# haoheliu/AudioLDM2

Hardware: AMD Instinct MI355X
Metric: audio_seconds_per_second (higher is better)
Workload: dtype f32 storage/accumulate; each product = 6 bf16 MFMA partial products of exact 3-part operand splits (fp32-grade); 1 GPU; audioldm2-full: batch 8 prompts/GPU x 1 GPU, 10.24 s @16 kHz, 200 DDIM steps, CFG 3.5, eta 1.0, n_candidates 1; one step = sample_log + VAE decode + HiFi-GAN + D2H of the waveform; synthetic conditioning, random-init weights, host-CPU RNG noise; global_batch=8, parallelism=prompt-sharded replicas x1, weight_broadcast_bytes=0

## Files before the change

### audioldm2_amd/csrc/api.hip

```cpp
#include "common.h"
#include <string.h>

namespace aldm {
static thread_local char g_err[512] = "";
void set_error(const char* fmt, ...) {
    va_list ap;
    va_start(ap, fmt);
    vsnprintf(g_err, sizeof(g_err), fmt, ap);
    va_end(ap);
}
}

extern "C" int aldm_version(void) { return 27; }
extern "C" const char* aldm_last_error(void) { return aldm::g_err; }
```

### audioldm2_amd/csrc/norm.hip

```cpp
#include <stdlib.h>
#include "igemm_epilogue.h"

namespace aldm {

constexpr int GN_ITERS = 16;
constexpr int GN_UNROLL = 8;

struct GnPart {
    float n, mean, m2;
};

__device__ __forceinline__ void gn_merge(double& n, double& mean, double& m2, double nb, double mb, double m2b) {
    if (nb <= 0.0) return;
    const double nt = n + nb;
    const double dlt = mb - mean;
    mean += dlt * (nb / nt);
    m2 += m2b + dlt * dlt * (n * nb / nt);
    n = nt;
}

template <bool FUSED>
__global__ __launch_bounds__(256) void gn_partial_kernel(const float* __restrict__ x1,
                                                         const float* __restrict__ x2, int P,
                                                         int C1, int C2, int G, int cols, int rows,
                                                         int chunk_px, float* __restrict__ ws, float eps,
                                                         const float* __restrict__ gamma,
                                                         const float* __restrict__ beta,
                                                         float* __restrict__ scale, float* __restrict__ shift, int gpb,
                                                         char* __restrict__ dst = nullptr, char* __restrict__ dst_raw = nullptr,
                                                         int parts = 3, int act = ALDM_ACT_NONE, int raw_parts = 3,
                                                         float f16_scale = 0.f) {
    const int C = C1 + C2;
    const int Cg4 = (C / G) >> 2;
    const int b = blockIdx.y;
    const int chunk = FUSED ? 0 : blockIdx.x;
    const int g_lo = FUSED ? blockIdx.x * gpb : 0;
    const int c4_lo = g_lo * Cg4, C4 = c4_lo + gpb * Cg4;
    const int p0 = chunk * chunk_px;
    const int p1 = min(P, p0 + chunk_px);
    const int tid = threadIdx.x;
    const int tx = tid % cols, ty = tid / cols;
    __shared__ GnPart ps[256];
    const int npass = (C4 - c4_lo + cols - 1) / cols;
    __shared__ double gacc[64][3];
    if (tid < 64) gacc[tid][0] = gacc[tid][1] = gacc[tid][2] = 0.0;
    __syncthreads();
    for (int cp = 0; cp < npass; ++cp) {
        const int c4 = c4_lo + cp * cols + tx;
        GnPart part = {0.f, 0.f, 0.f};
        if (ty < rows && c4 < C4 && p0 + ty < p1) {
            const int c = c4 << 2;
            const bool first = c < C1;
            const float* src = first ? x1 + (int64_t)b * P * C1 + c : x2 + (int64_t)b * P * C2 + (c - C1);
            const int pitch = first ? C1 : C2;
            float sa[GN_UNROLL], sq[GN_UNROLL];
#pragma unroll
            for (int u = 0; u < GN_UNROLL; ++u) sa[u] = sq[u] = 0.f;
            int p = p0 + ty;
            const f32x4 pv = *reinterpret_cast<const f32x4*>(src + (int64_t)p * pitch);
            const float pivot = fmaxf(fminf(pv[0], pv[1]), fminf(fmaxf(pv[0], pv[1]), pv[2]));
            int cnt = 0;
            for (; p + (GN_UNROLL - 1) * rows < p1; p += GN_UNROLL * rows) {
                f32x4 v[GN_UNROLL];
#pragma unroll
                for (int u = 0; u < GN_UNROLL; ++u)
                    v[u] = *reinterpret_cast<const f32x4*>(src + (int64_t)(p + u * rows) * pitch) - pivot;
#pragma unroll
                for (int u = 0; u < GN_UNROLL; ++u) {
                    sa[u] += (v[u][0] + v[u][1]) + (v[u][2] + v[u][3]);
                    sq[u] += (v[u][0] * v[u][0] + v[u][1] * v[u][1]) + (v[u][2] * v[u][2] + v[u][3] * v[u][3]);
                }
                cnt += GN_UNROLL;
            }
            for (; p < p1; p += rows) {
                const f32x4 v = *reinterpret_cast<const f32x4*>(src + (int64_t)p * pitch) - pivot;
                sa[0] += (v[0] + v[1]) + (v[2] + v[3]);
                sq[0] += (v[0] * v[0] + v[1] * v[1]) + (v[2] * v[2] + v[3] * v[3]);
                ++cnt;
            }
            float s = 0.f, ss = 0.f;
#pragma unroll
            for (int u = 0; u < GN_UNROLL; u += 2) {
                s += sa[u] + sa[u + 1];
                ss += sq[u] + sq[u + 1];
            }
            const float n = 4.0f * (float)cnt;
            const float md = s / n;
            part.n = n;
            part.mean = pivot + md;
            part.m2 = fmaxf(ss - s * md, 0.f);
        }
        if constexpr (FUSED) {
            __shared__ double wred[4][3];
            const int mygl = (c4 - c4_lo) / Cg4;
            for (int gl = 0; gl < gpb; ++gl) {
                const bool mine = part.n > 0.f && mygl == gl;
                double n = mine ? (double)part.n : 0.0, mean = mine ? (double)part.mean : 0.0, m2 = mine ? (double)part.m2 : 0.0;
#pragma unroll
                for (int o = 32; o > 0; o >>= 1) {
                    const double nb = __shfl_xor(n, o), mb = __shfl_xor(mean, o), m2b = __shfl_xor(m2, o);
                    gn_merge(n, mean, m2, nb, mb, m2b);
                }
                if ((tid & 63) == 0) {
                    wred[tid >> 6][0] = n;
                    wred[tid >> 6][1] = mean;
                    wred[tid >> 6][2] = m2;
                }
                __syncthreads();
                if (tid == 0) {
                    double an = gacc[gl][0], am = gacc[gl][1], a2 = gacc[gl][2];
                    for (int w = 0; w < 4; ++w) gn_merge(an, am, a2, wred[w][0], wred[w][1], wred[w][2]);
                    gacc[gl][0] = an;
                    gacc[gl][1] = am;
                    gacc[gl][2] = a2;
                }
                __syncthreads();
            }
            continue;
        }
        ps[tid] = part;
        __syncthreads();
        if (tid < gpb) {
            const int g = g_lo + tid;
            const int base = c4_lo + cp * cols;
            const int lo = max(g * Cg4, base), hi = min((g + 1) * Cg4, min(C4, base + cols));
            if (lo < hi) {
                double n = gacc[tid][0], mean = gacc[tid][1], m2 = gacc[tid][2];
                for (int yy = 0; yy < rows; ++yy)
                    for (int cc = lo; cc < hi; ++cc) {
                        const GnPart& t = ps[yy * cols + (cc - base)];
                        gn_merge(n, mean, m2, (double)t.n, (double)t.mean, (double)t.m2);
                    }
                gacc[tid][0] = n;
                gacc[tid][1] = mean;
                gacc[tid][2] = m2;
            }
        }
        __syncthreads();
    }
    if (FUSED) {
        const int Cg = C / G;
        __shared__ float fin[64][2];
        if (tid < gpb) {
            const double n = gacc[tid][0];
            double var = n > 0.0 ? gacc[tid][2] / n : 0.0;
            if (var < 0.0) var = 0.0;
            fin[tid][0] = (float)gacc[tid][1];
            fin[tid][1] = (float)(1.0 / sqrt(var + (double)eps));
        }
        __syncthreads();
        __shared__ float lsc[256], lsh[256];
        for (int c = g_lo * Cg + tid; c < (g_lo + gpb) * Cg; c += 256) {
            const int g = c / Cg - g_lo;
            const float sc = fin[g][1] * (gamma ? gamma[c] : 1.f);
            const float sh = (beta ? beta[c] : 0.f) - fin[g][0] * sc;
            scale[(int64_t)b * C + c] = sc;
            shift[(int64_t)b * C + c] = sh;
            if (dst) {
                lsc[c - g_lo * Cg] = sc;
                lsh[c - g_lo * Cg] = sh;
            }
        }
        if (dst) {
            __syncthreads();
            const int c_lo = g_lo * Cg, sw = (gpb * Cg) >> 3;
            for (int i = tid; i < P * sw; i += 256) {
                const int p = i / sw;
                const int cl = (i - p * sw) << 3;
                const int c = c_lo + cl;
                const int64_t row = (int64_t)b * P + p;
                const float* src = c < C1 ? x1 + row * C1 + c : x2 + row * C2 + (c - C1);
                f32x4 v0 = *reinterpret_cast<const f32x4*>(src);
                f32x4 v1 = *reinterpret_cast<const f32x4*>(src + 4);
                const int64_t off = (row * (C >> 5) + (c >> 5)) * (64 * parts) + (c & 31) * 2;
                u32x2 p0[3], p1[3];
                if (dst_raw) {
                    const int64_t roff = (row * (C >> 5) + (c >> 5)) * (64 * raw_parts) + (c & 31) * 2;
                    split4_parts(v0, p0, raw_parts);
                    split4_parts(v1, p1, raw_parts);
#pragma unroll
                    for (int q = 0; q < 3; ++q)
                        if (q < raw_parts)
                            *reinterpret_cast<u32x4*>(dst_raw + roff + q * 64) = u32x4{p0[q][0], p0[q][1], p1[q][0], p1[q][1]};
                }
#pragma unroll
                for (int e = 0; e < 4; ++e) {
                    v0[e] = __builtin_fmaf(v0[e], lsc[cl + e], lsh[cl + e]);
                    v1[e] = __builtin_fmaf(v1[e], lsc[cl + 4 + e], lsh[cl + 4 + e]);
                }
                if (act == ALDM_ACT_SILU) {
#pragma unroll
                    for (int e = 0; e < 4; ++e) {
                        v0[e] = silu_fast(v0[e]);
                        v1[e] = silu_fast(v1[e]);
                    }
                }
                split4_fmt(v0, p0, parts, f16_scale);
                split4_fmt(v1, p1, parts, f16_scale);
#pragma unroll
                for (int q = 0; q < 3; ++q)
                    if (q < parts) *reinterpret_cast<u32x4*>(dst + off + q * 64) = u32x4{p0[q][0], p0[q][1], p1[q][0], p1[q][1]};
            }
        }
    } else if (tid < G) {
// ... 217 lines not shown
        pl.cols = c4b < 256 ? c4b : 256;
        pl.rows = 256 / pl.cols;
        pl.chunk_px = P;
        pl.chunks = 1;
        pl.passes = (c4b + pl.cols - 1) / pl.cols;
    } else {
        pl.form = ALDM_GN_CHUNKED;
        gn_geometry(P, C, &pl.cols, &pl.rows, &pl.chunk_px, &pl.chunks);
        pl.passes = (C / 4 + pl.cols - 1) / pl.cols;
    }
    const int px = P < pl.chunk_px ? P : pl.chunk_px;
    pl.active = pl.cols * (pl.rows < px ? pl.rows : px);
    return pl;
}

}

using namespace aldm;

extern "C" int64_t aldm_gn_ws_floats(int B, int P, int C, int G) {
    int cols, rows, chunk_px, chunks;
    gn_geometry(P, C, &cols, &rows, &chunk_px, &chunks);
    return (int64_t)B * chunks * G * 6 + 2;
}

extern "C" int aldm_split_rows(const float* x1, const float* x2, int C1, int C2, int64_t rows, int P, const float* scale,
                               const float* shift, int act, void* dst, void* dst_raw, int parts, void* stream);
extern "C" int aldm_split_rows_f16(const float* x1, const float* x2, int C1, int C2, int64_t rows, int P, const float* scale,
                                   const float* shift, int act, float slope, void* dst, void* dst_raw, int raw_parts, float f16_scale,
                                   void* stream);

extern "C" int aldm_groupnorm_plan(int B, int P, int C1, int C2, int G, int want_split, int* form, int* group_slices,
                                   int* groups_per_block, int* chunks, int* chunk_px, int* cols, int* rows, int* passes,
                                   int* active_threads) {
    const int C = C1 + C2;
    ALDM_CHECK(B > 0 && P > 0 && C1 > 0 && C2 >= 0, "aldm_groupnorm_plan: bad shape (B=%d P=%d C1=%d C2=%d)", B, P, C1, C2);
    ALDM_CHECK(G > 0 && G <= 64 && C % G == 0 && (C / G) % 4 == 0 && C1 % 4 == 0,
               "aldm_groupnorm_plan: need C%%G==0, (C/G)%%4==0, C1%%4==0 (C1=%d C2=%d G=%d)", C1, C2, G);
    ALDM_CHECK(!want_split || (C % 32 == 0 && C1 % 8 == 0 && C2 % 8 == 0),
               "aldm_groupnorm_plan: a split image needs (C1+C2) %% 32 == 0, C1 %% 8 == 0 (C1=%d C2=%d)", C1, C2);
    const GnPlan pl = groupnorm_plan(B, P, C, C1, G, want_split != 0);
    if (form) *form = pl.form;
    if (group_slices) *group_slices = pl.gs;
    if (groups_per_block) *groups_per_block = pl.gpb;
    if (chunks) *chunks = pl.chunks;
    if (chunk_px) *chunk_px = pl.chunk_px;
    if (cols) *cols = pl.cols;
    if (rows) *rows = pl.rows;
    if (passes) *passes = pl.passes;
    if (active_threads) *active_threads = pl.active;
    return 0;
}

static int groupnorm_launch(const float* x1, const float* x2, int B, int P, int C1, int C2, int G, float eps,
                            const float* gamma, const float* beta, float* scale, float* shift, float* ws, void* dst,
                            void* dst_raw, int parts, int act, void* stream, int raw_parts = 0, float f16_scale = 0.f) {
    if (raw_parts == 0) raw_parts = parts;
    if (!x2) C2 = 0;
    const int C = C1 + C2;
    ALDM_CHECK(x1 && scale && shift && ws, "aldm_groupnorm_stats: null pointer");
    ws = reinterpret_cast<float*>((reinterpret_cast<uintptr_t>(ws) + 7) & ~uintptr_t(7));
    ALDM_CHECK(G > 0 && G <= 64 && C % G == 0 && (C / G) % 4 == 0 && C1 % 4 == 0,
               "aldm_groupnorm_stats: need C%%G==0, (C/G)%%4==0, C1%%4==0 (C1=%d C2=%d G=%d)", C1, C2, G);
    const GnPlan pl = groupnorm_plan(B, P, C, C1, G, dst != nullptr);
    hipStream_t st = (hipStream_t)stream;
    if (pl.form == ALDM_GN_FUSED_SPLIT) {
        hipLaunchKernelGGL(gn_partial_kernel<true>, dim3(pl.gs, B), dim3(256), 0, st, x1, x2, P, C1, C2, G, pl.cols, pl.rows, P, ws,
                           eps, gamma, beta, scale, shift, pl.gpb, reinterpret_cast<char*>(dst),
                           reinterpret_cast<char*>(dst_raw), parts, act, raw_parts, f16_scale);
        ALDM_LAUNCH_CHECK("aldm_groupnorm_split");
        return 0;
    }
    if (pl.form == ALDM_GN_FUSED) {
        hipLaunchKernelGGL(gn_partial_kernel<true>, dim3(pl.gs, B), dim3(256), 0, st, x1, x2, P, C1, C2, G, pl.cols,
                           pl.rows, P, ws, eps, gamma, beta, scale, shift, pl.gpb, nullptr, nullptr, 3, ALDM_ACT_NONE);
    } else {
        hipLaunchKernelGGL(gn_partial_kernel<false>, dim3(pl.chunks, B), dim3(256), 0, st, x1, x2, P, C1, C2, G,
                           pl.cols, pl.rows, pl.chunk_px, ws, eps, gamma, beta, scale, shift, G);
        hipLaunchKernelGGL(gn_finalize_kernel, dim3(B), dim3(256), 0, st, ws, pl.chunks, P, C, G, eps, gamma,
                           beta, scale, shift);
    }
    ALDM_LAUNCH_CHECK("aldm_groupnorm_stats");
    if (dst) {
        if (f16_scale != 0.f)
            return aldm_split_rows_f16(x1, x2, C1, C2, (int64_t)B * P, P, scale, shift, act, 0.f, dst, dst_raw, raw_parts, f16_scale, stream);
        return aldm_split_rows(x1, x2, C1, C2, (int64_t)B * P, P, scale, shift, act, dst, dst_raw, parts, stream);
    }
    return 0;
}

extern "C" int aldm_groupnorm_stats(const float* x1, const float* x2, int B, int P, int C1, int C2,
                                    int G, float eps, const float* gamma, const float* beta,
                                    float* scale, float* shift, float* ws, void* stream) {
    return groupnorm_launch(x1, x2, B, P, C1, C2, G, eps, gamma, beta, scale, shift, ws, nullptr, nullptr, 3, ALDM_ACT_NONE,
                            stream);
}

extern "C" int aldm_groupnorm_split(const float* x1, const float* x2, int B, int P, int C1, int C2, int G, float eps,
                                    const float* gamma, const float* beta, int act, float* scale, float* shift, float* ws,
                                    void* dst, void* dst_raw, int parts, void* stream) {
    if (!x2) C2 = 0;
    ALDM_CHECK(dst != nullptr && (parts == 2 || parts == 3) && (C1 + C2) % 32 == 0 && C1 % 8 == 0 && C2 % 8 == 0,
               "aldm_groupnorm_split: need dst, parts 2|3, (C1+C2) %% 32 == 0, C1 %% 8 == 0 (C1=%d C2=%d)", C1, C2);
    ALDM_CHECK(act == ALDM_ACT_NONE || act == ALDM_ACT_SILU, "aldm_groupnorm_split: activation %d not supported", act);
    ALDM_CHECK(((reinterpret_cast<uintptr_t>(dst) | reinterpret_cast<uintptr_t>(dst_raw)) & 15) == 0,
               "aldm_groupnorm_split: split images must be 16-byte aligned");
    return groupnorm_launch(x1, x2, B, P, C1, C2, G, eps, gamma, beta, scale, shift, ws, dst, dst_raw, parts, act, stream);
}

extern "C" int aldm_groupnorm_split_f16(const float* x1, const float* x2, int B, int P, int C1, int C2, int G, float eps,
                                        const float* gamma, const float* beta, int act, float* scale, float* shift, float* ws,
                                        void* dst, void* dst_raw, int raw_parts, float f16_scale, void* stream) {
    if (!x2) C2 = 0;
    ALDM_CHECK(dst != nullptr && f16_scale > 0.0f && (raw_parts == 2 || raw_parts == 3) && (C1 + C2) % 32 == 0 && C1 % 8 == 0 && C2 % 8 == 0,
               "aldm_groupnorm_split_f16: need dst, f16_scale > 0, raw_parts 2|3, (C1+C2) %% 32 == 0, C1 %% 8 == 0 (C1=%d C2=%d)", C1, C2);
    ALDM_CHECK(act == ALDM_ACT_NONE || act == ALDM_ACT_SILU, "aldm_groupnorm_split_f16: activation %d not supported", act);
    ALDM_CHECK(((reinterpret_cast<uintptr_t>(dst) | reinterpret_cast<uintptr_t>(dst_raw)) & 15) == 0,
               "aldm_groupnorm_split_f16: split images must be 16-byte aligned");
    return groupnorm_launch(x1, x2, B, P, C1, C2, G, eps, gamma, beta, scale, shift, ws, dst, dst_raw, 2, act, stream, raw_parts, f16_scale);
}

static int layernorm_launch(const float* x, float* y, void* y_split, int parts, int M, int C, const float* gamma,
                            const float* beta, float eps, void* stream, const char* name, bool rms = false, float f16_scale = 0.f) {
    ALDM_CHECK(parts == 2 || parts == 3, "%s: parts must be 2 or 3", name);
    ALDM_CHECK(x && (y || y_split) && gamma && (beta || rms), "%s: null pointer", name);
    ALDM_CHECK(C % 4 == 0 && C <= 256 * LN_MAXV, "%s: C=%d must be a multiple of 4 and <= %d", name, C, 256 * LN_MAXV);
    ALDM_CHECK(y_split == nullptr || (C % 32 == 0 && (reinterpret_cast<uintptr_t>(y_split) & 15) == 0),
               "%s: a split-image output needs C %% 32 == 0 and 16-byte alignment", name);
    hipStream_t st = (hipStream_t)stream;
#define ALDM_LN(V_, R_)                                                                                             \
    do {                                                                                                            \
        if (rms)                                                                                                    \
            hipLaunchKernelGGL((layernorm_kernel<V_, R_, true>), dim3(cdiv(M, 4 * R_)), dim3(256), 0, st, x, y, M, C, \
                               gamma, beta, eps, y_split, parts, f16_scale);                                        \
// ... 80 lines not shown
```

### audioldm2_amd/lib.py

```python
from __future__ import annotations

import ctypes as C
import os

_HERE = os.path.dirname(os.path.abspath(__file__))
LIB_PATH = os.environ.get("ALDM_LIB_PATH") or os.path.join(_HERE, "libaldm_hip.so")
ABI_VERSION = 27

ACT_NONE, ACT_SILU, ACT_LRELU, ACT_TANH, ACT_LOGCLAMP, ACT_GELU, ACT_GELU_TANH = range(7)
B_PACKED, B_NT = 0, 1
EPI_PLAIN, EPI_GEGLU, EPI_QKV = 0, 1, 2
GN_CHUNKED, GN_FUSED, GN_FUSED_SPLIT = 0, 1, 2
FMT_BF16, FMT_F16 = 0, 1
EPI_FORM_GENERIC, EPI_FORM_PLAIN, EPI_FORM_ROWBIAS, EPI_FORM_RES = range(4)


class IgemmDesc(C.Structure):

    _fields_ = [
        ("x1", C.c_void_p), ("x2", C.c_void_p),
        ("C1", C.c_int32), ("C2", C.c_int32),
        ("pix1", C.c_int32), ("pix2", C.c_int32),
        ("B", C.c_int32), ("H", C.c_int32), ("W", C.c_int32),
        ("up_h", C.c_int32), ("up_w", C.c_int32),
        ("KH", C.c_int32), ("KW", C.c_int32), ("SH", C.c_int32), ("SW", C.c_int32),
        ("PH", C.c_int32), ("PW", C.c_int32), ("DH", C.c_int32), ("DW", C.c_int32),
        ("OH", C.c_int32), ("OW", C.c_int32),
        ("pre_scale", C.c_void_p), ("pre_shift", C.c_void_p),
        ("pre_act", C.c_int32), ("pre_slope", C.c_float),
        ("w", C.c_void_p),
        ("b_mode", C.c_int32), ("ldb", C.c_int32),
        ("K", C.c_int32), ("N", C.c_int32),
        ("bias", C.c_void_p), ("rowbias", C.c_void_p), ("res", C.c_void_p), ("out", C.c_void_p),
        ("ldo", C.c_int32), ("act", C.c_int32), ("act_slope", C.c_float), ("alpha", C.c_float),
        ("accumulate", C.c_int32),
        ("out_mul", C.c_int32), ("out_off", C.c_int32), ("out_len", C.c_int32),
        ("batch", C.c_int32),
        ("stride_x", C.c_int64), ("stride_w", C.c_int64), ("stride_o", C.c_int64),
        ("rowbias_ld", C.c_int32), ("epi_mode", C.c_int32),
        ("ws", C.c_void_p), ("ws_floats", C.c_int64),
        ("hint_bm", C.c_int32), ("hint_bn", C.c_int32), ("hint_splits", C.c_int32), ("hint_kgroups", C.c_int32),
        ("w_split", C.c_void_p), ("hint_mma", C.c_int32), ("hint_stages", C.c_int32),
        ("a_split", C.c_void_p), ("out_split", C.c_void_p), ("out_split_c", C.c_int32), ("split_parts", C.c_int32),
        ("out_split_act", C.c_int32), ("out_split_slope", C.c_float),
        ("k_split", C.c_void_p), ("vt_split", C.c_void_p), ("qkv_c", C.c_int32), ("qkv_rows", C.c_int32),
        ("a_fmt", C.c_int32), ("acc_scale", C.c_float), ("out_split_parts", C.c_int32),
        ("out_split_fmt", C.c_int32), ("out_split_scale", C.c_float), ("vt_scale", C.c_float),
    ]


MAX_WINDOWS = 32


class WindowStarts(C.Structure):

    _fields_ = [("n", C.c_int), ("s", C.c_int * MAX_WINDOWS)]


MAX_ROWS = 64


class WindowRows(C.Structure):

    _fields_ = [("n", C.c_int), ("s", C.c_int * MAX_ROWS)]


_SIGS = {
    "aldm_version": (C.c_int, []),
    "aldm_last_error": (C.c_char_p, []),
    "aldm_igemm": (C.c_int, [C.POINTER(IgemmDesc), C.c_void_p]),
    "aldm_igemm_plan": (C.c_int, [C.POINTER(IgemmDesc), C.POINTER(C.c_int), C.POINTER(C.c_int),
                                  C.POINTER(C.c_int64), C.POINTER(C.c_int), C.POINTER(C.c_int),
                                  C.POINTER(C.c_int)]),
    "aldm_igemm_ws_floats": (C.c_int64, [C.POINTER(IgemmDesc)]),
    "aldm_igemm_plan_stages": (C.c_int, [C.POINTER(IgemmDesc)]),
    "aldm_igemm_plan_epilogue": (C.c_int, [C.POINTER(IgemmDesc)]),
    "aldm_igemm_epilogue_forms": (C.c_int, [C.c_int]),
    "aldm_igemm_force": (None, [C.c_int, C.c_int, C.c_int, C.c_int]),
    "aldm_igemm_force_stages": (None, [C.c_int]),
    "aldm_igemm_wave8_mask": (C.c_int, [C.c_int]),
    "aldm_split_image_bytes": (C.c_int64, [C.c_int64, C.c_int, C.c_int]),
    "aldm_split_rows": (C.c_int, [C.c_void_p, C.c_void_p, C.c_int, C.c_int, C.c_int64, C.c_int, C.c_void_p, C.c_void_p,
                                  C.c_int, C.c_void_p, C.c_void_p, C.c_int, C.c_void_p]),
    "aldm_split_rows_act": (C.c_int, [C.c_void_p, C.c_void_p, C.c_int, C.c_int, C.c_int64, C.c_int, C.c_void_p, C.c_void_p,
                                      C.c_int, C.c_float, C.c_void_p, C.c_void_p, C.c_int, C.c_void_p]),
    "aldm_layernorm_split": (C.c_int, [C.c_void_p, C.c_void_p, C.c_void_p, C.c_int, C.c_int, C.c_void_p, C.c_void_p,
                                       C.c_float, C.c_int, C.c_void_p]),
    "aldm_attention_d32_split": (C.c_int, [C.c_void_p, C.c_void_p, C.c_void_p, C.c_void_p, C.c_void_p, C.c_int, C.c_int,
                                           C.c_int, C.c_int, C.c_int, C.c_int, C.c_int, C.c_int, C.c_int,
                                           C.c_void_p, C.c_float, C.c_void_p]),
    "aldm_split_bytes_parts": (C.c_int64, [C.c_int, C.c_int, C.c_int]),
    "aldm_pack_split_bf16_parts": (C.c_int, [C.c_void_p, C.c_void_p, C.c_int, C.c_int, C.c_int, C.c_void_p]),
    "aldm_pack_split_f16": (C.c_int, [C.c_void_p, C.c_void_p, C.c_int, C.c_int, C.c_float, C.c_void_p]),
    "aldm_split_rows_f16": (C.c_int, [C.c_void_p, C.c_void_p, C.c_int, C.c_int, C.c_int64, C.c_int, C.c_void_p, C.c_void_p,
                                      C.c_int, C.c_float, C.c_void_p, C.c_void_p, C.c_int, C.c_float, C.c_void_p]),
    "aldm_groupnorm_split_f16": (C.c_int, [C.c_void_p, C.c_void_p, C.c_int, C.c_int, C.c_int, C.c_int, C.c_int, C.c_float,
                                           C.c_void_p, C.c_void_p, C.c_int, C.c_void_p, C.c_void_p, C.c_void_p, C.c_void_p,
                                           C.c_void_p, C.c_int, C.c_float, C.c_void_p]),
    "aldm_layernorm_split_f16": (C.c_int, [C.c_void_p, C.c_void_p, C.c_void_p, C.c_int, C.c_int, C.c_void_p, C.c_void_p,
                                           C.c_float, C.c_float, C.c_void_p]),
    "aldm_igemm_mma": (C.c_int, [C.c_int]),
    "aldm_split_bytes": (C.c_int64, [C.c_int, C.c_int]),
    "aldm_pack_split_bf16": (C.c_int, [C.c_void_p, C.c_void_p, C.c_int, C.c_int, C.c_void_p]),
    "aldm_pack_weight": (C.c_int, [C.c_void_p, C.c_void_p, C.c_int, C.c_int, C.c_int, C.c_int,
                                   C.c_int, C.c_int, C.c_int, C.c_void_p]),
    "aldm_pack_kn": (C.c_int, [C.c_void_p, C.c_void_p, C.c_int, C.c_int, C.c_int, C.c_int,
                               C.c_int64, C.c_int64, C.c_void_p]),
    "aldm_groupnorm_stats": (C.c_int, [C.c_void_p, C.c_void_p, C.c_int, C.c_int, C.c_int, C.c_int,
                                       C.c_int, C.c_float, C.c_void_p, C.c_void_p, C.c_void_p,
                                       C.c_void_p, C.c_void_p, C.c_void_p]),
    "aldm_gn_ws_floats": (C.c_int64, [C.c_int, C.c_int, C.c_int, C.c_int]),
    "aldm_groupnorm_plan": (C.c_int, [C.c_int] * 6 + [C.POINTER(C.c_int)] * 9),
    "aldm_groupnorm_split": (C.c_int, [C.c_void_p, C.c_void_p, C.c_int, C.c_int, C.c_int, C.c_int, C.c_int, C.c_float,
                                       C.c_void_p, C.c_void_p, C.c_int, C.c_void_p, C.c_void_p, C.c_void_p, C.c_void_p,
                                       C.c_void_p, C.c_int, C.c_void_p]),
    "aldm_layernorm": (C.c_int, [C.c_void_p, C.c_void_p, C.c_int, C.c_int, C.c_void_p, C.c_void_p,
                                 C.c_float, C.c_void_p]),
    "aldm_attention_mma": (C.c_int, [C.c_int]),
    "aldm_attention_sched": (C.c_int, [C.c_int]),
    "aldm_attention_query_tiles": (C.c_int, [C.c_int, C.c_int, C.c_int]),
    "aldm_attention_d32_presplit_f16": (C.c_int, [C.c_void_p, C.c_void_p, C.c_void_p, C.c_void_p, C.c_void_p, C.c_int, C.c_float,
                                                  C.c_int, C.c_int, C.c_int, C.c_int, C.c_int, C.c_int, C.c_float, C.c_float,
                                                  C.c_float, C.c_float, C.c_void_p]),
    "aldm_attention_d32_presplit": (C.c_int, [C.c_void_p, C.c_void_p, C.c_void_p, C.c_void_p, C.c_void_p, C.c_int, C.c_int,
                                              C.c_int, C.c_int, C.c_int, C.c_int, C.c_int, C.c_float, C.c_void_p]),
    "aldm_vt_regroup": (C.c_int, [C.c_void_p, C.c_void_p, C.c_int, C.c_int, C.c_int, C.c_int, C.c_void_p]),
    "aldm_attention_d32": (C.c_int, [C.c_void_p, C.c_void_p, C.c_void_p, C.c_void_p, C.c_int,
                                     C.c_int, C.c_int, C.c_int, C.c_int, C.c_int, C.c_int, C.c_int,
                                     C.c_void_p, C.c_float, C.c_void_p]),
    "aldm_rel_attention": (C.c_int, [C.c_void_p, C.c_void_p, C.c_void_p, C.c_void_p, C.c_int, C.c_int, C.c_int, C.c_int,
                                     C.c_int, C.c_int, C.c_int, C.c_int, C.c_void_p, C.c_void_p, C.c_int, C.c_void_p,
                                     C.c_void_p]),
    "aldm_rowscale_add": (C.c_int, [C.c_void_p, C.c_void_p, C.c_void_p, C.c_void_p, C.c_int64, C.c_int, C.c_int, C.c_void_p]),
    "aldm_rmsnorm": (C.c_int, [C.c_void_p, C.c_void_p, C.c_int, C.c_int, C.c_void_p, C.c_float, C.c_void_p]),
    "aldm_softmax_rows_bias": (C.c_int, [C.c_void_p, C.c_void_p, C.c_int, C.c_int, C.c_int, C.c_int, C.c_float, C.c_void_p,
                                         C.c_void_p, C.c_void_p]),
    "aldm_resample_sinc": (C.c_int, [C.c_void_p, C.c_void_p, C.c_void_p, C.c_int, C.c_int, C.c_int, C.c_int, C.c_int, C.c_int,
                                     C.c_int, C.c_void_p]),
    "aldm_power_spec": (C.c_int, [C.c_void_p, C.c_void_p, C.c_int64, C.c_int, C.c_int, C.c_int, C.c_void_p]),
    "aldm_col_affine": (C.c_int, [C.c_void_p, C.c_void_p, C.c_void_p, C.c_void_p, C.c_int64, C.c_int, C.c_void_p]),
    "aldm_bicubic_patchify": (C.c_int, [C.c_void_p, C.c_void_p, C.c_int, C.c_int, C.c_int, C.c_int, C.c_int, C.c_void_p]),
    "aldm_token_mean": (C.c_int, [C.c_void_p, C.c_void_p, C.c_int, C.c_int, C.c_int, C.c_void_p]),
    "aldm_row_cosine": (C.c_int, [C.c_void_p, C.c_void_p, C.c_void_p, C.c_int, C.c_int, C.c_float, C.c_void_p]),
    "aldm_decode_linear": (C.c_int, [C.c_void_p, C.c_int, C.c_int, C.c_int, C.c_void_p, C.c_int, C.c_void_p, C.c_void_p,
                                     C.c_void_p, C.c_float, C.c_int, C.c_void_p, C.c_int, C.c_void_p, C.c_int, C.c_void_p]),
    "aldm_decode_attention": (C.c_int, [C.c_void_p, C.c_int, C.c_void_p, C.c_void_p, C.c_void_p, C.c_void_p, C.c_int, C.c_int,
                                        C.c_int, C.c_float, C.c_void_p, C.c_int, C.c_void_p]),
    "aldm_decode_gemv_slices": (C.c_int, [C.c_int, C.c_int]),
    "aldm_decode_gemv": (C.c_int, [C.c_void_p, C.c_int, C.c_int, C.c_int64, C.c_void_p, C.c_int, C.c_int, C.c_int, C.c_void_p,
                                   C.c_int, C.c_void_p, C.c_void_p]),
    "aldm_decode_reduce_ln": (C.c_int, [C.c_void_p, C.c_int, C.c_int64, C.c_int, C.c_void_p, C.c_void_p, C.c_void_p, C.c_int,
                                        C.c_int, C.c_int, C.c_void_p, C.c_int, C.c_void_p, C.c_void_p, C.c_float, C.c_void_p,
                                        C.c_int, C.c_void_p, C.c_int, C.c_void_p]),
    "aldm_decode_attention_parts": (C.c_int, [C.c_void_p, C.c_int, C.c_int, C.c_int64, C.c_void_p, C.c_void_p, C.c_void_p,
                                              C.c_void_p, C.c_void_p, C.c_int, C.c_int, C.c_int, C.c_float, C.c_void_p, C.c_int,
                                              C.c_void_p]),
    "aldm_softmax_rows_masked": (C.c_int, [C.c_void_p, C.c_void_p, C.c_int, C.c_int, C.c_int, C.c_int, C.c_float,
                                           C.c_void_p, C.c_int, C.c_void_p]),
    "aldm_softmax_rows": (C.c_int, [C.c_void_p, C.c_void_p, C.c_int64, C.c_int, C.c_float,
                                    C.c_void_p]),
    "aldm_geglu": (C.c_int, [C.c_void_p, C.c_void_p, C.c_int64, C.c_int, C.c_void_p]),
    "aldm_timestep_embedding": (C.c_int, [C.c_void_p, C.c_void_p, C.c_int, C.c_int, C.c_float,
                                          C.c_void_p]),
    "aldm_nchw_to_nhwc": (C.c_int, [C.c_void_p, C.c_void_p, C.c_int, C.c_int, C.c_int, C.c_int,
                                    C.c_void_p]),
# ... 136 lines not shown
```

### audioldm2_amd/ops.py

```python
from __future__ import annotations

import ctypes as C
import json
import os
from dataclasses import dataclass
from typing import List, Optional, Sequence, Tuple

import torch

from . import lib as _l
from .lib import (ACT_GELU, ACT_GELU_TANH, ACT_LOGCLAMP, ACT_LRELU, ACT_NONE, ACT_SILU, ACT_TANH, B_NT, B_PACKED,
                  IgemmDesc)


def _stream() -> int:
    return torch.cuda.current_stream().cuda_stream


def _p(t: Optional[torch.Tensor]):
    return None if t is None else t.data_ptr()


def _chk(t: torch.Tensor, name: str):
    if not (t.is_cuda and t.dtype == torch.float32 and t.is_contiguous()):
# ... 767 lines not shown
    _igemm(d, "igemm(nt)")
    return out


def pack_kn(src: torch.Tensor) -> torch.Tensor:
    sp, ss, lds = _view3(src, "pack_kn.src")
    Z, K, N = src.shape
    per = ((K + 3) // 4) * _npad(N) * 4
    dst = torch.empty((Z, per), device=src.device, dtype=torch.float32)
    _l.check(_l.load().aldm_pack_kn(sp, dst.data_ptr(), K, N, lds, Z, ss, per, _stream()), "pack_kn")
    return dst


def gemm_packed_batched(a: torch.Tensor, bp: torch.Tensor, K: int, N: int, *,
                        out: Optional[torch.Tensor] = None) -> torch.Tensor:
    _chk(a, "gemm_packed.a")
    Z, M, Ka = a.shape
    assert Ka == K and K % 4 == 0
    if out is None:
        out = torch.empty((Z, M, N), device=a.device, dtype=torch.float32)
    d = IgemmDesc()
    d.x1 = a.data_ptr(); d.C1 = K; d.B = 1; d.H = 1; d.W = M; d.up_h = d.up_w = 1
    d.KH = d.KW = d.SH = d.SW = d.DH = d.DW = 1
    d.OH = 1; d.OW = M
    d.w = bp.data_ptr(); d.b_mode = B_PACKED; d.ldb = 0; d.K = K; d.N = N
    d.out = out.data_ptr(); d.ldo = N; d.alpha = 1.0
    d.batch = Z; d.stride_x = M * K; d.stride_w = bp.shape[1]; d.stride_o = M * N
    _igemm(d, "igemm(packed batched)")
    return out


_gn_ws = {}


def gn_stats(x: torch.Tensor, gamma: torch.Tensor, beta: torch.Tensor, *, groups: int = 32,
             eps: float = 1e-5, x2: Optional[torch.Tensor] = None):
    _chk(x, "gn.x")
    B = x.shape[0]
    C1 = x.shape[-1]
    P = x.numel() // (B * C1)
    C2 = 0
    if x2 is not None:
        _chk(x2, "gn.x2")
        C2 = x2.shape[-1]
    Cc = C1 + C2
    lib = _l.load()
    nws = lib.aldm_gn_ws_floats(B, P, Cc, groups)
    ws = torch.empty(nws, device=x.device, dtype=torch.float32)
    ss = torch.empty((2, B, Cc), device=x.device, dtype=torch.float32)
    _l.check(lib.aldm_groupnorm_stats(x.data_ptr(), _p(x2), B, P, C1, C2, groups, eps,
                                      gamma.data_ptr(), beta.data_ptr(), ss[0].data_ptr(),
                                      ss[1].data_ptr(), ws.data_ptr(), _stream()), "groupnorm_stats")
    return ss[0], ss[1]


GN_FORMS = ("chunked", "fused", "fused_split")


def groupnorm_plan(B: int, P: int, C1: int, C2: int = 0, groups: int = 32, want_split: bool = False) -> dict:
    import ctypes
    out = [ctypes.c_int() for _ in range(9)]
    _l.check(_l.load().aldm_groupnorm_plan(B, P, C1, C2, groups, 1 if want_split else 0, *[ctypes.byref(o) for o in out]),
             "groupnorm_plan")
    keys = ("form", "group_slices", "groups_per_block", "chunks", "chunk_px", "cols", "rows", "passes", "active_threads")
    plan = {k: o.value for k, o in zip(keys, out)}
    plan["form"] = GN_FORMS[plan["form"]]
    return plan


def gn_split(x: torch.Tensor, gamma: torch.Tensor, beta: torch.Tensor, *, groups: int = 32, eps: float = 1e-5,
             x2: Optional[torch.Tensor] = None, act: int = ACT_NONE, want_raw: bool = False):
    _chk(x, "gn_split.x")
    B = x.shape[0]
    C1 = x.shape[-1]
    P = x.numel() // (B * C1)
    C2 = 0
    if x2 is not None:
        _chk(x2, "gn_split.x2")
        assert x2.shape[:-1] == x.shape[:-1]
        C2 = x2.shape[-1]
    Cc = C1 + C2
    lib = _l.load()
    ws = torch.empty(lib.aldm_gn_ws_floats(B, P, Cc, groups), device=x.device, dtype=torch.float32)
    ss = torch.empty((2, B, Cc), device=x.device, dtype=torch.float32)
    shape = (*x.shape[:-1], Cc)
    raw = SplitT.empty(shape, x.device) if want_raw else None
    if f16_mode():
        dst = SplitT.empty(shape, x.device, f16_scale=_norm_f16_scale(gamma, beta, (Cc // groups) * P))
        _l.check(lib.aldm_groupnorm_split_f16(x.data_ptr(), _p(x2), B, P, C1, C2, groups, eps, gamma.data_ptr(), beta.data_ptr(), act,
                                              ss[0].data_ptr(), ss[1].data_ptr(), ws.data_ptr(), dst.data_ptr(),
                                              None if raw is None else raw.data_ptr(), 3, dst.scale, _stream()), "groupnorm_split_f16")
        return (dst, raw) if want_raw else dst
    dst = SplitT.empty(shape, x.device)
    _l.check(lib.aldm_groupnorm_split(x.data_ptr(), _p(x2), B, P, C1, C2, groups, eps, gamma.data_ptr(), beta.data_ptr(), act,
                                      ss[0].data_ptr(), ss[1].data_ptr(), ws.data_ptr(), dst.data_ptr(),
                                      None if raw is None else raw.data_ptr(), dst.parts, _stream()), "groupnorm_split")
    return (dst, raw) if want_raw else dst


def layernorm(x: torch.Tensor, gamma: torch.Tensor, beta: torch.Tensor, eps: float = 1e-5,
              split_out: Optional[str] = None):
    _chk(x, "ln.x")
    Cc = x.shape[-1]
    M = x.numel() // Cc
    y = None if split_out == "only" else torch.empty_like(x)
    if not split_out:
# ... 894 lines not shown
```

### include/aldm_hip.h

```cpp
#ifndef ALDM_HIP_H
#define ALDM_HIP_H

#include <stdint.h>

#ifdef __cplusplus
extern "C" {
#endif

int aldm_version(void);
const char* aldm_last_error(void);

enum {
    ALDM_ACT_NONE = 0,
    ALDM_ACT_SILU = 1,
    ALDM_ACT_LRELU = 2,
    ALDM_ACT_TANH = 3,
    ALDM_ACT_LOGCLAMP = 4,
    ALDM_ACT_GELU = 5,
    ALDM_ACT_GELU_TANH = 6
};

enum { ALDM_EPI_PLAIN = 0, ALDM_EPI_GEGLU = 1, ALDM_EPI_QKV = 2 };

enum {
// ... 59 lines not shown
    float vt_scale;
} aldm_igemm_desc;

int aldm_igemm(const aldm_igemm_desc* d, void* stream);
int64_t aldm_igemm_ws_floats(const aldm_igemm_desc* d);
enum { ALDM_FMT_BF16 = 0, ALDM_FMT_F16 = 1 };
int aldm_igemm_plan(const aldm_igemm_desc* d, int* bm, int* bn, int64_t* flops, int* splits, int* kgroups,
                    int* mma);
int aldm_igemm_plan_stages(const aldm_igemm_desc* d);
enum { ALDM_EPI_FORM_GENERIC = 0, ALDM_EPI_FORM_PLAIN = 1, ALDM_EPI_FORM_ROWBIAS = 2, ALDM_EPI_FORM_RES = 3 };
int aldm_igemm_plan_epilogue(const aldm_igemm_desc* d);
int aldm_igemm_epilogue_forms(int on);
void aldm_igemm_force(int bm, int bn, int splits, int kgroups);
void aldm_igemm_force_stages(int stages);
int aldm_igemm_wave8_mask(int mask);
int aldm_igemm_mma(int mode);
#ifdef ALDM_TEST_HOOKS
int aldm_debug_drop_product(int on);
#endif
int64_t aldm_split_bytes(int K, int N);
int aldm_pack_split_bf16(const float* packed, void* dst, int K, int N, void* stream);
int64_t aldm_split_bytes_parts(int K, int N, int parts);
int aldm_pack_split_bf16_parts(const float* packed, void* dst, int K, int N, int parts, void* stream);
int aldm_pack_split_f16(const float* packed, void* dst, int K, int N, float scale, void* stream);

int64_t aldm_split_image_bytes(int64_t rows, int C, int parts);
int aldm_split_rows(const float* x1, const float* x2, int C1, int C2, int64_t rows, int P, const float* scale,
                    const float* shift, int act, void* dst, void* dst_raw, int parts, void* stream);
int aldm_split_rows_act(const float* x1, const float* x2, int C1, int C2, int64_t rows, int P, const float* scale,
                        const float* shift, int act, float slope, void* dst, void* dst_raw, int parts, void* stream);
int aldm_split_rows_f16(const float* x1, const float* x2, int C1, int C2, int64_t rows, int P, const float* scale,
                        const float* shift, int act, float slope, void* dst, void* dst_raw, int raw_parts, float f16_scale,
                        void* stream);

int aldm_pack_weight(const float* src, float* dst, int N, int Cin, int KH, int KW,
                     int transposed, int phase, int stride, void* stream);
int aldm_pack_kn(const float* src, float* dst, int K, int N, int lds, int batch,
                 int64_t stride_src, int64_t stride_dst, void* stream);

int aldm_groupnorm_stats(const float* x1, const float* x2, int B, int P, int C1, int C2,
                         int G, float eps, const float* gamma, const float* beta,
                         float* scale, float* shift, float* ws, void* stream);
int64_t aldm_gn_ws_floats(int B, int P, int C, int G);
enum { ALDM_GN_CHUNKED = 0, ALDM_GN_FUSED = 1, ALDM_GN_FUSED_SPLIT = 2 };
int aldm_groupnorm_plan(int B, int P, int C1, int C2, int G, int want_split, int* form, int* group_slices,
                        int* groups_per_block, int* chunks, int* chunk_px, int* cols, int* rows, int* passes,
                        int* active_threads);
int aldm_groupnorm_split(const float* x1, const float* x2, int B, int P, int C1, int C2, int G, float eps,
                         const float* gamma, const float* beta, int act, float* scale, float* shift, float* ws,
                         void* dst, void* dst_raw, int parts, void* stream);
int aldm_groupnorm_split_f16(const float* x1, const float* x2, int B, int P, int C1, int C2, int G, float eps,
                             const float* gamma, const float* beta, int act, float* scale, float* shift, float* ws,
                             void* dst, void* dst_raw, int raw_parts, float f16_scale, void* stream);
int aldm_layernorm(const float* x, float* y, int M, int C, const float* gamma,
                   const float* beta, float eps, void* stream);
int aldm_layernorm_split(const float* x, float* y, void* y_split, int M, int C, const float* gamma,
                         const float* beta, float eps, int parts, void* stream);
int aldm_layernorm_split_f16(const float* x, float* y, void* y_split, int M, int C, const float* gamma,
                             const float* beta, float eps, float f16_scale, void* stream);

int aldm_attention_d32(const float* q, const float* k, const float* v, float* out,
                       int B, int heads, int Lq, int Lk, int ldq, int ldk, int ldv, int ldo,
                       const float* mask, float scale, void* stream);
int aldm_attention_d32_split(const float* q, const float* k, const float* v, float* out, void* out_split,
                             int parts, int B, int heads, int Lq, int Lk, int ldq, int ldk, int ldv, int ldo,
                             const float* mask, float scale, void* stream);
int aldm_attention_d32_presplit(const float* q, const void* k_split, const void* vt_split, float* out, void* out_split,
                                int parts, int B, int heads, int Lq, int Lk, int ldq, int ldo, float scale, void* stream);
int aldm_vt_regroup(const void* src, void* dst, int B, int L, int heads, int parts, void* stream);
int aldm_attention_mma(int mode);
int aldm_attention_sched(int sched);
int aldm_attention_query_tiles(int B, int heads, int Lq);
int aldm_attention_d32_presplit_f16(const float* q, const void* k_split, const void* vt_split, float* out, void* out_split,
                                    int out_parts, float out_scale, int B, int heads, int Lq, int Lk, int ldq, int ldo,
                                    float scale, float q_scale, float k_scale, float v_scale, void* stream);
int aldm_xattn_fold_plan(int B, int L, int C, int heads, int Lk, int* tile_rows, int* col_splits, int* waves, int* blocks,
                         int* lds_bytes);
int64_t aldm_xattn_fold_bytes(int B, int C);
int aldm_xattn_fold_prepare(const float* kv, const float* wq, const float* wout, void* mq_img, void* mo_img, int B, int C,
                            int heads, int Lk, void* stream);
int aldm_xattn_folded(const float* h, float* out, const float* gamma, const float* beta, float eps, const void* mq_img,
                      const void* mo_img, const float* b_out, const float* mask, int B, int L, int C, int heads, int Lk,
                      void* stream);
int aldm_rel_attention(const float* q, const float* k, const float* v, float* out, int B, int heads, int T, int d,
                       int ldq, int ldk, int ldv, int ldo, const float* emb_k, const float* emb_v, int window,
                       const float* mask, void* stream);
int aldm_rowscale_add(const float* x, const float* s, const float* res, float* y, int64_t rows, int C, int divide,
                      void* stream);
int aldm_rmsnorm(const float* x, float* y, int M, int C, const float* weight, float eps, void* stream);
int aldm_softmax_rows_bias(const float* x, float* y, int B, int heads, int q_rows, int N, float scale, const float* bias,
                           const float* keymask, void* stream);
int aldm_softmax_rows(const float* x, float* y, int64_t M, int N, float scale, void* stream);
int aldm_softmax_rows_masked(const float* x, float* y, int B, int heads, int q_rows, int N, float scale,
                             const float* keymask, int q_pos0, void* stream);

int aldm_decode_linear(const float* x, int ldx, int M, int K, const float* w_kn, int N, const float* bias,
                       const float* ln_gamma, const float* ln_beta, float ln_eps, int act, const float* res, int ldr,
                       float* y, int ldy, void* stream);
int aldm_decode_attention(const float* qkv, int ldq, const int64_t* pos, float* k_cache, float* v_cache, const float* keymask,
                          int B, int heads, int n_tot, float scale, float* out, int ldo, void* stream);
int aldm_decode_gemv_slices(int K, int N);
int aldm_decode_gemv(const float* x, int ldx, int xparts, int64_t xstride, const float* xbias, int xact, int M, int K,
                     const float* w_kn, int N, float* ypart, void* stream);
int aldm_decode_reduce_ln(const float* part, int nparts, int64_t pstride, int ldp, const float* bias, const int64_t* bias_row,
                          const float* res, int ldr, int M, int N, float* h_out, int ldh, const float* ln_gamma,
                          const float* ln_beta, float ln_eps, float* xn, int ldn, float* xn2, int ldn2, void* stream);
// ... 96 lines not shown
```

Baseline: 19.69 audio-s/s.

## Add fast fused GroupNorm path with prefetched loads and batched group reductions

```diff
diff --git a/audioldm2_amd/csrc/api.hip b/audioldm2_amd/csrc/api.hip
--- a/audioldm2_amd/csrc/api.hip
+++ b/audioldm2_amd/csrc/api.hip
@@ -11,5 +11,5 @@
 }
 }
 
-extern "C" int aldm_version(void) { return 27; }
+extern "C" int aldm_version(void) { return 28; }
 extern "C" const char* aldm_last_error(void) { return aldm::g_err; }
diff --git a/audioldm2_amd/csrc/norm.hip b/audioldm2_amd/csrc/norm.hip
--- a/audioldm2_amd/csrc/norm.hip
+++ b/audioldm2_amd/csrc/norm.hip
@@ -1,4 +1,5 @@
 #include <stdlib.h>
+#include <atomic>
 #include "igemm_epilogue.h"
 
 namespace aldm {
@@ -19,7 +20,22 @@
     n = nt;
 }
 
-template <bool FUSED>
+__device__ __forceinline__ void gn_merge_sel(double& n, double& mean, double& m2, double nb, double mb, double m2b) {
+    const bool keep = nb <= 0.0;
+    double n_ = n, mean_ = mean, m2_ = m2;
+    const double nt = n_ + nb;
+    const double dlt = mb - mean_;
+    mean_ += dlt * (nb / nt);
+    m2_ += m2b + dlt * dlt * (n_ * nb / nt);
+    n_ = nt;
+    n = keep ? n : n_;
+    mean = keep ? mean : mean_;
+    m2 = keep ? m2 : m2_;
+}
+
+constexpr int GN_APPLY_U = 4;
+
+template <bool FUSED, int FAST = 0>
 __global__ __launch_bounds__(256) void gn_partial_kernel(const float* __restrict__ x1,
                                                          const float* __restrict__ x2, int P,
                                                          int C1, int C2, int G, int cols, int rows,
@@ -45,6 +61,26 @@
     __shared__ double gacc[64][3];
     if (tid < 64) gacc[tid][0] = gacc[tid][1] = gacc[tid][2] = 0.0;
     __syncthreads();
+    const int c_lo = g_lo * (C / G), c_hi = (g_lo + gpb) * (C / G), sw = (c_hi - c_lo) >> 3, nit = P * sw;
+    const int c_pre = min(c_lo + tid, c_hi - 1);
+    float ga_pre = 1.f, be_pre = 0.f;
+    f32x4 ap_v0[GN_APPLY_U], ap_v1[GN_APPLY_U];
+    int ap_p[GN_APPLY_U], ap_cl[GN_APPLY_U];
+    auto apply_load = [&](int base) {
+#pragma unroll
+        for (int k = 0; k < GN_APPLY_U; ++k) {
+            const int i = min(base + tid + 256 * k, nit - 1);
+            const int p = i / sw;
+            const int cl = (i - p * sw) << 3;
+            const int c = c_lo + cl;
+            const int64_t row = (int64_t)b * P + p;
+            const float* src = c < C1 ? x1 + row * C1 + c : x2 + row * C2 + (c - C1);
+            ap_v0[k] = *reinterpret_cast<const f32x4*>(src);
+            ap_v1[k] = *reinterpret_cast<const f32x4*>(src + 4);
+            ap_p[k] = p;
+            ap_cl[k] = cl;
+        }
+    };
     for (int cp = 0; cp < npass; ++cp) {
         const int c4 = c4_lo + cp * cols + tx;
         GnPart part = {0.f, 0.f, 0.f};
@@ -57,9 +93,45 @@
 #pragma unroll
             for (int u = 0; u < GN_UNROLL; ++u) sa[u] = sq[u] = 0.f;
             int p = p0 + ty;
+            float pivot;
+            int cnt = 0;
+            if constexpr (FAST != 0) {
+                int left = (p1 - 1 - p) / rows + 1;
+                const int plast = p + (left - 1) * rows;
+                f32x4 v[GN_UNROLL];
+#pragma unroll
+                for (int u = 0; u < GN_UNROLL; ++u)
+                    v[u] = *reinterpret_cast<const f32x4*>(src + (int64_t)min(p + u * rows, plast) * pitch);
+                pivot = fmaxf(fminf(v[0][0], v[0][1]), fminf(fmaxf(v[0][0], v[0][1]), v[0][2]));
+                while (left >= GN_UNROLL) {
+#pragma unroll
+                    for (int u = 0; u < GN_UNROLL; ++u) v[u] = v[u] - pivot;
+#pragma unroll
+                    for (int u = 0; u < GN_UNROLL; ++u) {
+                        sa[u] += (v[u][0] + v[u][1]) + (v[u][2] + v[u][3]);
+                        sq[u] += (v[u][0] * v[u][0] + v[u][1] * v[u][1]) + (v[u][2] * v[u][2] + v[u][3] * v[u][3]);
+                    }
+                    cnt += GN_UNROLL;
+                    left -= GN_UNROLL;
+                    p += GN_UNROLL * rows;
+                    if (left > 0) {
+#pragma unroll
+                        for (int u = 0; u < GN_UNROLL; ++u)
+                            v[u] = *reinterpret_cast<const f32x4*>(src + (int64_t)min(p + u * rows, plast) * pitch);
+                    }
+                }
+#pragma unroll
+                for (int u = 0; u < GN_UNROLL - 1; ++u) {
+                    if (u < left) {
+                        const f32x4 w = v[u] - pivot;
+                        sa[0] += (w[0] + w[1]) + (w[2] + w[3]);
+                        sq[0] += (w[0] * w[0] + w[1] * w[1]) + (w[2] * w[2] + w[3] * w[3]);
+                        ++cnt;
+                    }
+                }
+            } else {
             const f32x4 pv = *reinterpret_cast<const f32x4*>(src + (int64_t)p * pitch);
-            const float pivot = fmaxf(fminf(pv[0], pv[1]), fminf(fmaxf(pv[0], pv[1]), pv[2]));
-            int cnt = 0;
+            pivot = fmaxf(fminf(pv[0], pv[1]), fminf(fmaxf(pv[0], pv[1]), pv[2]));
             for (; p + (GN_UNROLL - 1) * rows < p1; p += GN_UNROLL * rows) {
                 f32x4 v[GN_UNROLL];
 #pragma unroll
@@ -78,6 +150,7 @@
                 sq[0] += (v[0] * v[0] + v[1] * v[1]) + (v[2] * v[2] + v[3] * v[3]);
                 ++cnt;
             }
+            }
             float s = 0.f, ss = 0.f;
 #pragma unroll
             for (int u = 0; u < GN_UNROLL; u += 2) {
@@ -90,7 +163,47 @@
             part.mean = pivot + md;
             part.m2 = fmaxf(ss - s * md, 0.f);
         }
-        if constexpr (FUSED) {
+        if constexpr (FUSED && FAST != 0) {
+            if (cp == 0) {
+                if (dst) apply_load(0);
+                ga_pre = gamma ? gamma[c_pre] : 1.f;
+                be_pre = beta ? beta[c_pre] : 0.f;
+            }
+            __shared__ double wredf[4][FAST][3];
+            const int mygl = (c4 - c4_lo) / Cg4;
+            double n[FAST], mean[FAST], m2[FAST];
+#pragma unroll
+            for (int gl = 0; gl < FAST; ++gl) {
+                const bool mine = part.n > 0.f && mygl == gl;
+                n[gl] = mine ? (double)part.n : 0.0, mean[gl] = mine ? (double)part.mean : 0.0, m2[gl] = mine ? (double)part.m2 : 0.0;
+            }
+#pragma unroll
+            for (int o = 32; o > 0; o >>= 1) {
+                double nb[FAST], mb[FAST], m2b[FAST];
+#pragma unroll
+                for (int gl = 0; gl < FAST; ++gl) nb[gl] = __shfl_xor(n[gl], o), mb[gl] = __shfl_xor(mean[gl], o), m2b[gl] = __shfl_xor(m2[gl], o);
+#pragma unroll
+                for (int gl = 0; gl < FAST; ++gl) gn_merge_sel(n[gl], mean[gl], m2[gl], nb[gl], mb[gl], m2b[gl]);
+            }
+            if ((tid & 63) == 0) {
+#pragma unroll
+                for (int gl = 0; gl < FAST; ++gl) {
+                    wredf[tid >> 6][gl][0] = n[gl];
+                    wredf[tid >> 6][gl][1] = mean[gl];
+                    wredf[tid >> 6][gl][2] = m2[gl];
+                }
+            }
+            __syncthreads();
+            if (tid < FAST) {
+                double an = gacc[tid][0], am = gacc[tid][1], a2 = gacc[tid][2];
+                for (int w = 0; w < 4; ++w) gn_merge(an, am, a2, wredf[w][tid][0], wredf[w][tid][1], wredf[w][tid][2]);
+                gacc[tid][0] = an;
+                gacc[tid][1] = am;
+                gacc[tid][2] = a2;
+            }
+            __syncthreads();
+            continue;
+        } else if constexpr (FUSED) {
             __shared__ double wred[4][3];
             const int mygl = (c4 - c4_lo) / Cg4;
             for (int gl = 0; gl < gpb; ++gl) {
@@ -150,6 +263,69 @@
         }
         __syncthreads();
         __shared__ float lsc[256], lsh[256];
+        if constexpr (FAST != 0) {
+            for (int c = c_lo + tid; c < c_hi; c += 256) {
+                const int g = c / Cg - g_lo;
+                const bool pre = c == c_pre;
+                const float sc = fin[g][1] * (pre ? ga_pre : gamma ? gamma[c] : 1.f);
+                const float sh = (pre ? be_pre : beta ? beta[c] : 0.f) - fin[g][0] * sc;
+                scale[(int64_t)b * C + c] = sc;
+                shift[(int64_t)b * C + c] = sh;
+                if (dst) {
+                    lsc[c - c_lo] = sc;
+                    lsh[c - c_lo] = sh;
+                }
+            }
+            if (dst) {
+                __syncthreads();
+                for (int base = 0; base < nit; base += 256 * GN_APPLY_U) {
+                    f32x4 t0[GN_APPLY_U], t1[GN_APPLY_U];
+                    int tp[GN_APPLY_U], tcl[GN_APPLY_U];
+#pragma unroll
+                    for (int k = 0; k < GN_APPLY_U; ++k) t0[k] = ap_v0[k], t1[k] = ap_v1[k], tp[k] = ap_p[k], tcl[k] = ap_cl[k];
+                    if (base + 256 * GN_APPLY_U < nit) apply_load(base + 256 * GN_APPLY_U);
+#pragma unroll
+                    for (int k = 0; k < GN_APPLY_U; ++k) {
+                        if (base + tid + 256 * k >= nit) continue;
+                        const int p = tp[k];
+                        const int cl = tcl[k];
+                        const int c = c_lo + cl;
+                        const int64_t row = (int64_t)b * P + p;
+                        f32x4 v0 = t0[k];
+                        f32x4 v1 = t1[k];
+                        const int64_t off = (row * (C >> 5) + (c >> 5)) * (64 * parts) + (c & 31) * 2;
+                        u32x2 p0[3], p1[3];
+                        if (dst_raw) {
+                            const int64_t roff = (row * (C >> 5) + (c >> 5)) * (64 * raw_parts) + (c & 31) * 2;
+                            split4_parts(v0, p0, raw_parts);
+                            split4_parts(v1, p1, raw_parts);
+#pragma unroll
+                            for (int q = 0; q < 3; ++q)
+                                if (q < raw_parts)
+                                    *reinterpret_cast<u32x4*>(dst_raw + roff + q * 64) = u32x4{p0[q][0], p0[q][1], p1[q][0], p1[q][1]};
+                        }
+#pragma unroll
+                        for (int e = 0; e < 4; ++e) {
+                            v0[e] = __builtin_fmaf(v0[e], lsc[cl + e], lsh[cl + e]);
+                            v1[e] = __builtin_fmaf(v1[e], lsc[cl + 4 + e], lsh[cl + 4 + e]);
+                        }
+                        if (act == ALDM_ACT_SILU) {
+#pragma unroll
+                            for (int e = 0; e < 4; ++e) {
+                                v0[e] = silu_fast(v0[e]);
+                                v1[e] = silu_fast(v1[e]);
+                            }
+                        }
+                        split4_fmt(v0, p0, parts, f16_scale);
+                        split4_fmt(v1, p1, parts, f16_scale);
+#pragma unroll
+                        for (int q = 0; q < 3; ++q)
+                            if (q < parts) *reinterpret_cast<u32x4*>(dst + off + q * 64) = u32x4{p0[q][0], p0[q][1], p1[q][0], p1[q][1]};
+                    }
+                }
+            }
+            return;
+        }
         for (int c = g_lo * Cg + tid; c < (g_lo + gpb) * Cg; c += 256) {
             const int g = c / Cg - g_lo;
             const float sc = fin[g][1] * (gamma ? gamma[c] : 1.f);
@@ -473,6 +649,25 @@
     return 0;
 }
 
+static std::atomic<int> g_gn_fast{-1};
+static int gn_fast_on() {
+    static const int env_on = [] {
+        const char* e = getenv("ALDM_GN_FAST");
+        return (e && e[0] == '0' && e[1] == 0) ? 0 : 1;
+    }();
+    const int v = g_gn_fast.load(std::memory_order_relaxed);
+    return v < 0 ? env_on : v;
+}
+extern "C" int aldm_groupnorm_fast(int on) {
+    const int prev = gn_fast_on();
+    g_gn_fast.store(on == 0 || on == 1 ? on : -1, std::memory_order_relaxed);
+    return prev;
+}
+
+static bool gn_fast_shape(const GnPlan& pl) {
+    return gn_fast_on() && pl.form != ALDM_GN_CHUNKED && pl.gpb >= 1 && pl.gpb <= 4;
+}
+
 static int groupnorm_launch(const float* x1, const float* x2, int B, int P, int C1, int C2, int G, float eps,
                             const float* gamma, const float* beta, float* scale, float* shift, float* ws, void* dst,
                             void* dst_raw, int parts, int act, void* stream, int raw_parts = 0, float f16_scale = 0.f) {
@@ -485,22 +680,33 @@
                "aldm_groupnorm_stats: need C%%G==0, (C/G)%%4==0, C1%%4==0 (C1=%d C2=%d G=%d)", C1, C2, G);
     const GnPlan pl = groupnorm_plan(B, P, C, C1, G, dst != nullptr);
     hipStream_t st = (hipStream_t)stream;
+    const bool fast = gn_fast_shape(pl);
+#define ALDM_GN_FUSED_LAUNCH(K_, dst_, raw_, parts_, act_)                                                                     \
+    hipLaunchKernelGGL(K_, dim3(pl.gs, B), dim3(256), 0, st, x1, x2, P, C1, C2, G, pl.cols, pl.rows, P, ws, eps, gamma, beta, \
+                       scale, shift, pl.gpb, dst_, raw_, parts_, act_, raw_parts, f16_scale)
+#define ALDM_GN_FUSED_FORM(dst_, raw_, parts_, act_)                                                             \
+    do {                                                                                                         \
+        if (!fast) ALDM_GN_FUSED_LAUNCH((gn_partial_kernel<true>), dst_, raw_, parts_, act_);                    \
+        else if (pl.gpb == 1) ALDM_GN_FUSED_LAUNCH((gn_partial_kernel<true, 1>), dst_, raw_, parts_, act_);      \
+        else if (pl.gpb == 2) ALDM_GN_FUSED_LAUNCH((gn_partial_kernel<true, 2>), dst_, raw_, parts_, act_);      \
+        else if (pl.gpb == 3) ALDM_GN_FUSED_LAUNCH((gn_partial_kernel<true, 3>), dst_, raw_, parts_, act_);      \
+        else ALDM_GN_FUSED_LAUNCH((gn_partial_kernel<true, 4>), dst_, raw_, parts_, act_);                       \
+    } while (0)
     if (pl.form == ALDM_GN_FUSED_SPLIT) {
-        hipLaunchKernelGGL(gn_partial_kernel<true>, dim3(pl.gs, B), dim3(256), 0, st, x1, x2, P, C1, C2, G, pl.cols, pl.rows, P, ws,
-                           eps, gamma, beta, scale, shift, pl.gpb, reinterpret_cast<char*>(dst),
-                           reinterpret_cast<char*>(dst_raw), parts, act, raw_parts, f16_scale);
+        ALDM_GN_FUSED_FORM(reinterpret_cast<char*>(dst), reinterpret_cast<char*>(dst_raw), parts, act);
         ALDM_LAUNCH_CHECK("aldm_groupnorm_split");
         return 0;
     }
     if (pl.form == ALDM_GN_FUSED) {
-        hipLaunchKernelGGL(gn_partial_kernel<true>, dim3(pl.gs, B), dim3(256), 0, st, x1, x2, P, C1, C2, G, pl.cols,
-                           pl.rows, P, ws, eps, gamma, beta, scale, shift, pl.gpb, nullptr, nullptr, 3, ALDM_ACT_NONE);
+        ALDM_GN_FUSED_FORM((char*)nullptr, (char*)nullptr, 3, ALDM_ACT_NONE);
     } else {
         hipLaunchKernelGGL(gn_partial_kernel<false>, dim3(pl.chunks, B), dim3(256), 0, st, x1, x2, P, C1, C2, G,
                            pl.cols, pl.rows, pl.chunk_px, ws, eps, gamma, beta, scale, shift, G);
         hipLaunchKernelGGL(gn_finalize_kernel, dim3(B), dim3(256), 0, st, ws, pl.chunks, P, C, G, eps, gamma,
                            beta, scale, shift);
     }
+#undef ALDM_GN_FUSED_FORM
+#undef ALDM_GN_FUSED_LAUNCH
     ALDM_LAUNCH_CHECK("aldm_groupnorm_stats");
     if (dst) {
         if (f16_scale != 0.f)
diff --git a/audioldm2_amd/lib.py b/audioldm2_amd/lib.py
--- a/audioldm2_amd/lib.py
+++ b/audioldm2_amd/lib.py
@@ -5,7 +5,7 @@
 
 _HERE = os.path.dirname(os.path.abspath(__file__))
 LIB_PATH = os.environ.get("ALDM_LIB_PATH") or os.path.join(_HERE, "libaldm_hip.so")
-ABI_VERSION = 27
+ABI_VERSION = 28
 
 ACT_NONE, ACT_SILU, ACT_LRELU, ACT_TANH, ACT_LOGCLAMP, ACT_GELU, ACT_GELU_TANH = range(7)
 B_PACKED, B_NT = 0, 1
@@ -111,6 +111,7 @@
                                        C.c_void_p, C.c_void_p, C.c_void_p]),
     "aldm_gn_ws_floats": (C.c_int64, [C.c_int, C.c_int, C.c_int, C.c_int]),
     "aldm_groupnorm_plan": (C.c_int, [C.c_int] * 6 + [C.POINTER(C.c_int)] * 9),
+    "aldm_groupnorm_fast": (C.c_int, [C.c_int]),
     "aldm_groupnorm_split": (C.c_int, [C.c_void_p, C.c_void_p, C.c_int, C.c_int, C.c_int, C.c_int, C.c_int, C.c_float,
                                        C.c_void_p, C.c_void_p, C.c_int, C.c_void_p, C.c_void_p, C.c_void_p, C.c_void_p,
                                        C.c_void_p, C.c_int, C.c_void_p]),
diff --git a/audioldm2_amd/ops.py b/audioldm2_amd/ops.py
--- a/audioldm2_amd/ops.py
+++ b/audioldm2_amd/ops.py
@@ -843,6 +843,10 @@
                                       gamma.data_ptr(), beta.data_ptr(), ss[0].data_ptr(),
                                       ss[1].data_ptr(), ws.data_ptr(), _stream()), "groupnorm_stats")
     return ss[0], ss[1]
+
+
+def gn_fast(on: int = -1) -> int:
+    return _l.load().aldm_groupnorm_fast(on)
 
 
 GN_FORMS = ("chunked", "fused", "fused_split")
diff --git a/include/aldm_hip.h b/include/aldm_hip.h
--- a/include/aldm_hip.h
+++ b/include/aldm_hip.h
@@ -135,6 +135,7 @@
 int aldm_groupnorm_split_f16(const float* x1, const float* x2, int B, int P, int C1, int C2, int G, float eps,
                              const float* gamma, const float* beta, int act, float* scale, float* shift, float* ws,
                              void* dst, void* dst_raw, int raw_parts, float f16_scale, void* stream);
+int aldm_groupnorm_fast(int on);
 int aldm_layernorm(const float* x, float* y, int M, int C, const float* gamma,
                    const float* beta, float eps, void* stream);
 int aldm_layernorm_split(const float* x, float* y, void* y_split, int M, int C, const float* gamma,
```

Result: no change. 19.68 audio-s/s (-0.1%).
